# furkanyesiler/acoss

Hardware: AMD Instinct MI355X
Metric: track-pairs/sec on N x N Serra09 Qmax (HPCP, T=2000) (higher is better)
Workload: dtype f32

## Files before the change

acoss_amd/csrc/acx.hip:

```cpp
#include <hip/hip_runtime.h>

#include <chrono>
#include <dlfcn.h>
#include <rccl/rccl.h>

#include <algorithm>
#include <cmath>
#include <cstdio>
#include <cstdlib>
#include <cstring>
#include <string>
#include <vector>

#include "../../include/acx.h"
#include "serra09_kernels.hpp"
#include "serra09_long_kernels.hpp"
#include "serra09_locate_kernels.hpp"
#include "prep_kernels.hpp"
#include "snf_kernels.hpp"
#include "simple_kernels.hpp"
#include "ef_kernels.hpp"
#include "ef_rowstat2_kernels.hpp"
#include "ef_gemm_dma_kernels.hpp"
#include "ef_prep_kernels.hpp"
#include "ftm2d_kernels.hpp"
#include "rank_kernels.hpp"
#include "query_kernels.hpp"
#include "grid.hpp"
#include "serra09_plan.hpp"
#include "device_buffer.hpp"

using acx::PairDesc;
using acx::DeviceBuffer;
using acx::PinnedBuffer;

namespace {

std::string g_create_error;

struct KStat {
    const char *name;
    double ms;
    int64_t launches;
    int64_t cells;
};
enum { KS_OTI = 0, KS_NORMS, KS_BAND, KS_CSM, KS_SEL, KS_QMAX, KS_SIMPLE, KS_EFGEMM, KS_EFSTAT, KS_EFFUSE, KS_EFSW, KS_RANK, KS_TOPK, KS_FTMTILE, KS_QROWS, KS_QTOPK, KS_QRANK, KS_QTOPKL, KS_FTMPAIRS, KS_LOCATE, KS_COUNT };

struct PendingEvent {
    hipEvent_t a, b;
    int stat;
    int64_t cells;
};

struct Serra09Slot {
    std::vector<PairDesc> pd, sorted;
    std::vector<int> perm;
    DeviceBuffer<PairDesc> d_pd;
    DeviceBuffer<float> d_out;
    PinnedBuffer<float> h_out;
    PinnedBuffer<int64_t> h_idx;
    DeviceBuffer<int64_t> d_idx;
    hipEvent_t done = nullptr;
    hipEvent_t cls_ev[8] = {nullptr, nullptr, nullptr, nullptr, nullptr, nullptr, nullptr, nullptr};
    bool busy = false;
    bool on_q = false;
    int B = 0, w = 1;
    int64_t k0 = 0;
    DeviceBuffer<acx_alignment> d_al;
    PinnedBuffer<acx_alignment> h_al;
    std::vector<int64_t> seam_off;
    DeviceBuffer<int64_t> d_seam_off;
    bool al = false;
};

}

struct acx_ctx {
    int device = 0;
    hipStream_t stream = nullptr;
    hipStream_t qstream = nullptr;
    hipStream_t qstream2 = nullptr;
    hipEvent_t q2_done = nullptr;
    std::string err;
    float *d_frames0 = nullptr;
    int64_t *d_toff0 = nullptr;
    std::vector<int64_t> h_off0;
    int pool_tau = 0;
    float *d_frames = nullptr;
    float *d_frot = nullptr;
    _Float16 *d_fh = nullptr;
    float *d_normtab = nullptr;
    int64_t *d_noff = nullptr;
    int normtab_m = 0, normtab_span = -1;
    std::vector<int64_t> h_noff;
    int64_t *d_toff = nullptr;
    float *d_gch = nullptr;
    std::vector<int64_t> h_off;
    int32_t n_tracks = 0, dim = 0;
    DeviceBuffer<double> d_frames64;
    DeviceBuffer<int64_t> d_toff64;
    DeviceBuffer<double> d_prof64;
    DeviceBuffer<double> d_wn64;
    int wn64_L = 0;
    std::vector<int64_t> h_off64;
    int32_t n_tracks64 = 0;
    DeviceBuffer<int32_t> d_pairs;
    DeviceBuffer<double> d_out64;
    float *d_ef[3] = {nullptr, nullptr, nullptr};
    unsigned short *d_efs[3] = {nullptr, nullptr, nullptr};
    int ef_kp[3] = {0, 0, 0};
    float *d_efn[2] = {nullptr, nullptr};
    double *d_efmed = nullptr;
    int64_t *d_efoff = nullptr;
    std::vector<int64_t> h_efoff;
    int32_t ef_ntracks = 0;
    int32_t ef_gemm = ACX_EF_GEMM_DEFAULT;
// ... 551 lines not shown
            if ((int64_t)d.Mq * d.Mr + acx::LOC_STRIP >= ((int64_t)1 << 32))
                return fail(c, ACX_ERR_UNSUPPORTED, "serra09_align: pair " + std::to_string(k) + " has 2^32 cells or more");
        }
    }
    for (int s = 0; s < 2; ++s) {
        if (!c->slot[s].done) ACX_HIP(c, hipEventCreateWithFlags(&c->slot[s].done, hipEventDisableTiming));
        if (c->slot[s].busy) { ACX_HIP(c, hipEventSynchronize(c->slot[s].done)); c->slot[s].busy = false; }
    }

    int64_t k0 = 0;
    for (int batch = 0; k0 < K; ++batch) {
        Serra09Slot &S = c->slot[batch & 1];
        if ((rc = collect_slot(c, S, out, al)) != ACX_OK) return rc;
        std::vector<PairDesc> &pd = S.pd;
        acx::Serra09Arena used;
        const int64_t k = acx::serra09_pack_batch(len, pairs, k0, K, p, dbg != nullptr, limit_floats, pd, used);
        if (k == k0) return fail(c, ACX_ERR_STATE, "serra09: the batch plan made no progress at pair " + std::to_string(k0));
        const int B = (int)pd.size();
        const acx::Serra09Sort srt = acx::serra09_sort_batch(pd, S.sorted, S.perm, p.m);
        const int *key_begin = srt.key_begin, *cls_begin = srt.cls_begin;
        const std::vector<int> &perm = S.perm;
        if (cls_begin[NC] > 0 && (rc = ensure_normtab(c, p)) != ACX_OK) return rc;
        if (cls_begin[NC] > 0 && p.arith == ACX_ARITH_F16X2 && (rc = ensure_f16pool(c)) != ACX_OK) return rc;
        if ((rc = ensure(c, c->d_scratch, (size_t)std::max<int64_t>(used.scratch, 1))) != ACX_OK) return rc;
        if ((rc = ensure(c, c->d_bits, (size_t)std::max<int64_t>(used.bits, 1))) != ACX_OK) return rc;
        if ((rc = ensure(c, c->d_thr, (size_t)used.thr + 64 * 32 + 16)) != ACX_OK) return rc;
        if ((rc = ensure(c, S.d_pd, (size_t)B)) != ACX_OK) return rc;
        if ((rc = ensure(c, S.d_out, (size_t)2 * B)) != ACX_OK) return rc;
        if ((rc = ensure(c, S.h_out, (size_t)2 * B)) != ACX_OK) return rc;
        ACX_HIP(c, hipMemcpyAsync(S.d_pd, pd.data(), sizeof(PairDesc) * B, hipMemcpyHostToDevice, c->stream));
        if (al) {
            int64_t seams = 0;
            S.seam_off.resize((size_t)B);
            for (int k2 = 0; k2 < B; ++k2) { S.seam_off[(size_t)k2] = seams; seams += acx::loc_seam_records(pd[k2].Mq, pd[k2].Mr, p.dp_start); }
            if ((rc = ensure(c, S.d_al, (size_t)B)) != ACX_OK) return rc;
            if ((rc = ensure(c, S.h_al, (size_t)B)) != ACX_OK) return rc;
            if ((rc = ensure(c, S.d_seam_off, (size_t)B)) != ACX_OK) return rc;
            if ((rc = ensure(c, c->d_seam, (size_t)std::max<int64_t>(seams, 1))) != ACX_OK) return rc;
            ACX_HIP(c, hipMemcpyAsync(S.d_seam_off, S.seam_off.data(), sizeof(int64_t) * B, hipMemcpyHostToDevice, c->stream));
        }
        if (dd) {
            if ((rc = ensure(c, S.h_idx, (size_t)B)) != ACX_OK) return rc;
            if ((rc = ensure(c, S.d_idx, (size_t)B)) != ACX_OK) return rc;
            for (int k2 = 0; k2 < B; ++k2) S.h_idx[k2] = dd->idx[k0 + perm[k2]];
            ACX_HIP(c, hipMemcpyAsync(S.d_idx, S.h_idx, sizeof(int64_t) * B, hipMemcpyHostToDevice, c->stream));
        }
        const bool use_q = acx::serra09_switches().qstream && !dbg && !al && !c->prof && cls_begin[NC + 1] == cls_begin[NC];
        if (use_q && !c->qstream) ACX_HIP(c, hipStreamCreateWithFlags(&c->qstream, hipStreamNonBlocking));
        if (use_q && both && !c->qstream2) {
            ACX_HIP(c, hipStreamCreateWithFlags(&c->qstream2, hipStreamNonBlocking));
            ACX_HIP(c, hipEventCreateWithFlags(&c->q2_done, hipEventDisableTiming));
        }
        hipStream_t qs = use_q ? c->qstream : c->stream;
        if (use_q)
            for (int cl = 0; cl < NC; ++cl)
                if (!S.cls_ev[cl]) ACX_HIP(c, hipEventCreateWithFlags(&S.cls_ev[cl], hipEventDisableTiming));
        Serra09Slot &Sprev = c->slot[(batch & 1) ^ 1];
        bool bits_free = !(Sprev.busy && Sprev.on_q);

        {
            ProfScope ps(c, KS_OTI, acx::serra09_extent(pd, 0, B).cells);
            hipLaunchKernelGGL(acx::oti_kernel, dim3((B + 255) / 256), dim3(256), 0, c->stream,
                               S.d_pd, B, c->d_gch, p.oti, p.oti_target, c->d_toff, c->d_noff);
        }
        int64_t cls_cells[NC + 1];
        for (int cl = 0; cl <= NC; ++cl) {
            cls_cells[cl] = 0;
            const int b0 = cls_begin[cl], Bc = cls_begin[cl + 1] - b0;
            if (Bc <= 0) continue;
            const acx::Serra09Extent ce = acx::serra09_extent(pd, b0, b0 + Bc);
            cls_cells[cl] = ce.cells;
            if (cl < NC) {
                bool ok = true;
                for (int cq = 0; cq < NC; ++cq) {
                    const int q0 = key_begin[NC * cl + cq], Bq = key_begin[NC * cl + cq + 1] - q0;
                    if (Bq <= 0) continue;
                    const acx::Serra09Extent qe = acx::serra09_extent(pd, q0, q0 + Bq);
                    ProfScope ps(c, KS_BAND, qe.cells);
                    ok = ok && launch_band(c, p.m, S.d_pd + q0, Bq, qe.Mr, cq, p, 1, 0, dbg ? 1 : 0);
                }
                if (!bits_free) { ACX_HIP(c, hipStreamWaitEvent(c->stream, Sprev.done, 0)); bits_free = true; }
                {
                    ProfScope ps(c, KS_BAND, ce.cells);
                    ok = ok && launch_band(c, p.m, S.d_pd + b0, Bc, ce.Mq, cl, p, 0, dbg ? 1 : 0, dbg ? 1 : 0);
                }
                if (use_q) ACX_HIP(c, hipEventRecord(S.cls_ev[cl], c->stream));
                if (!ok) return fail(c, ACX_ERR_UNSUPPORTED, "serra09: this build of libacx has no band kernel for the requested m");
            } else {
                if (!bits_free) { ACX_HIP(c, hipStreamWaitEvent(c->stream, Sprev.done, 0)); bits_free = true; }
                launch_streaming_class(c, S.d_pd + b0, &pd[b0], Bc, ce, p);
            }
        }
        {
            hipError_t wait_err = hipSuccess;
            auto sweep = [&](bool dmax, float *dst, hipStream_t qs) {
                for (int cl = 0; cl <= NC; ++cl) {
                    const int b0 = cls_begin[cl], Bc = cls_begin[cl + 1] - b0;
                    if (Bc <= 0) continue;
                    if (use_q) { const hipError_t e_ = hipStreamWaitEvent(qs, S.cls_ev[cl], 0); if (e_ != hipSuccess) wait_err = e_; }
                    ProfScope ps(c, KS_QMAX, cls_cells[cl], qs);
                    const acx::Serra09Sweep sw = acx::serra09_sweep(cl);
                    launch_qmax_sweep(qs, S.d_pd + b0, Bc, c->d_bits, c->d_scratch, dst + (size_t)b0 * w, w, p.gamma_o, p.gamma_e, p.dp_start, dmax,
                                      sw.cols, sw.pack);
                }
            };
            if (al) {
                ProfScope ps(c, KS_LOCATE, acx::serra09_extent(pd, 0, B).cells, qs);
                launch_qmax_locate(qs, S.d_pd, B, c->d_bits, c->d_seam, S.d_seam_off, S.d_al, p.gamma_o, p.gamma_e, p.dp_start);
            } else if (both && use_q) {
                sweep(false, S.d_out, qs);
                sweep(true, S.d_out + 1, c->qstream2);
                ACX_HIP(c, hipEventRecord(c->q2_done, c->qstream2));
                ACX_HIP(c, hipStreamWaitEvent(qs, c->q2_done, 0));
            } else if (both) { sweep(false, S.d_out, qs); sweep(true, S.d_out + 1, qs); }
            else sweep(p.dmax != 0, S.d_out, qs);
            ACX_HIP(c, wait_err);
        }
        ACX_LAUNCHES_OK(c);
        if (al) {
            ACX_HIP(c, hipMemcpyAsync(S.h_al, S.d_al, sizeof(acx_alignment) * B, hipMemcpyDeviceToHost, qs));
        } else if (dd) {
            hipLaunchKernelGGL(scatter_scores_kernel, dim3((B + 255) / 256), dim3(256), 0, qs,
                               S.d_out, S.d_idx, dd->base, B, w);
            ACX_HIP(c, hipGetLastError());
        } else {
            ACX_HIP(c, hipMemcpyAsync(S.h_out, S.d_out, sizeof(float) * B * w, hipMemcpyDeviceToHost, qs));
        }
        ACX_HIP(c, hipEventRecord(S.done, qs));
        S.busy = true; S.on_q = use_q; S.B = B; S.w = w; S.k0 = k0; S.al = al != nullptr;

        if (dbg && B >= 1) {
            if ((rc = collect_slot(c, S, out)) != ACX_OK) return rc;
            PairDesc d;
            ACX_HIP(c, hipMemcpy(&d, S.d_pd, sizeof(PairDesc), hipMemcpyDeviceToHost));
            if (dbg->oti) *dbg->oti = d.oti;
            if (dbg->dims) { dbg->dims[0] = d.Mq; dbg->dims[1] = d.Mr; }
            if (dbg->d2)
                ACX_HIP(c, hipMemcpy2D(dbg->d2, sizeof(float) * d.Mr, c->d_scratch + d.offD, sizeof(float) * d.pitchD,
                                       sizeof(float) * d.Mr, d.Mq, hipMemcpyDeviceToHost));
            const float *X = c->d_thr + d.offX;
            if (dbg->thrq) ACX_HIP(c, hipMemcpy(dbg->thrq, X, sizeof(float) * d.Mq, hipMemcpyDeviceToHost));
            if (dbg->thrr) ACX_HIP(c, hipMemcpy(dbg->thrr, X + d.pitchT, sizeof(float) * d.Mr, hipMemcpyDeviceToHost));
            if (dbg->epsq) ACX_HIP(c, hipMemcpy(dbg->epsq, X + d.pitchT + d.pitchD, sizeof(float) * d.Mq, hipMemcpyDeviceToHost));
            if (dbg->epsr) ACX_HIP(c, hipMemcpy(dbg->epsr, X + 2 * d.pitchT + d.pitchD, sizeof(float) * d.Mr, hipMemcpyDeviceToHost));
        }
        k0 = k;
    }
    for (int s = 0; s < 2; ++s)
        if ((rc = collect_slot(c, c->slot[s], out, al)) != ACX_OK) return rc;
    return ACX_OK;
}

}


struct EfDebug { float *csm, *fused; int32_t *oti; int64_t which = 0; };
// ... 580 lines not shown
int acx_abi_version(void) { return ACX_ABI_VERSION; }

int acx_hip_versions(int *build, int *runtime)
{
    if (build) *build = HIP_VERSION;
    int v = 0;
    if (runtime) *runtime = hipRuntimeGetVersion(&v) == hipSuccess ? v : 0;
    return 0;
}

acx_ctx *acx_create(int device, int *err)
{
    auto bad = [&](int code, const std::string &msg) -> acx_ctx * {
        g_create_error = msg;
        if (err) *err = code;
        return nullptr;
    };
    int n = 0;
    hipError_t e = hipGetDeviceCount(&n);
    if (e != hipSuccess || n <= 0) return bad(ACX_ERR_HIP, std::string("no HIP device: ") + hipGetErrorString(e));
    if (device < 0 || device >= n) return bad(ACX_ERR_INVALID, "device index out of range");
    if ((e = hipSetDevice(device)) != hipSuccess) return bad(ACX_ERR_HIP, std::string("hipSetDevice: ") + hipGetErrorString(e));
    hipDeviceProp_t prop;
    if ((e = hipGetDeviceProperties(&prop, device)) != hipSuccess) return bad(ACX_ERR_HIP, std::string("hipGetDeviceProperties: ") + hipGetErrorString(e));
    if (std::string(prop.gcnArchName).rfind("gfx950", 0) != 0)
        return bad(ACX_ERR_HIP, std::string("libacx is built for gfx950 only; device is ") + prop.gcnArchName);
    acx_ctx *c = new acx_ctx();
    c->device = device;
    c->total_mem = prop.totalGlobalMem;
    c->n_cu = prop.multiProcessorCount;
    if ((e = hipStreamCreateWithFlags(&c->stream, hipStreamNonBlocking)) != hipSuccess) {
        delete c;
        return bad(ACX_ERR_HIP, std::string("hipStreamCreate: ") + hipGetErrorString(e));
    }
    if (err) *err = ACX_OK;
    return c;
}

static void comm_release(acx_ctx *c);
static void ftm2d_free_pool(acx_ctx *c);

void acx_destroy(acx_ctx *c)
{
    if (!c) return;
    (void)hipSetDevice(c->device);
    (void)hipStreamSynchronize(c->stream);
    if (c->qstream) (void)hipStreamSynchronize(c->qstream);
    if (c->qstream2) (void)hipStreamSynchronize(c->qstream2);
    comm_release(c);
    drain_profile(c);
    for (hipEvent_t ev : c->event_pool) (void)hipEventDestroy(ev);
    for (Serra09Slot &sl : c->slot) {
        if (sl.done) (void)hipEventDestroy(sl.done);
        for (hipEvent_t ev : sl.cls_ev)
            if (ev) (void)hipEventDestroy(ev);
    }
    for (hipEvent_t ev : c->rank_ev)
        if (ev) (void)hipEventDestroy(ev);
    if (c->q2_done) (void)hipEventDestroy(c->q2_done);
    if (c->qstream) (void)hipStreamDestroy(c->qstream);
    if (c->qstream2) (void)hipStreamDestroy(c->qstream2);
    (void)hipStreamDestroy(c->stream);
    free_pool(c);
    ef_free_pool(c);
    ftm2d_free_pool(c);
    delete c;
}

#ifdef ACX_EF_TIMING
extern "C" int acx_ef_clk(unsigned long long *out, int reset)
{
    if (out && hipMemcpyFromSymbol(out, HIP_SYMBOL(acx::g_ef_clk), sizeof(unsigned long long) * 16) != hipSuccess) return -1;
    if (reset) {
        unsigned long long z[16] = {0};
        if (hipMemcpyToSymbol(HIP_SYMBOL(acx::g_ef_clk), z, sizeof(z)) != hipSuccess) return -1;
    }
    return 0;
}
#endif

const char *acx_last_error(const acx_ctx *c) { return c ? c->err.c_str() : g_create_error.c_str(); }

int acx_set_scratch_limit(acx_ctx *c, int64_t bytes)
{
    if (!c) return ACX_ERR_INVALID;
    c->scratch_limit = bytes < 0 ? 0 : bytes;
    return ACX_OK;
}

int acx_set_nonfinite_policy(acx_ctx *c, int32_t policy)
{
    if (!c) return ACX_ERR_INVALID;
    if (policy != ACX_NONFINITE_REJECT && policy != ACX_NONFINITE_ZERO) return fail(c, ACX_ERR_INVALID, "set_nonfinite_policy: unknown policy");
    c->nonfinite_policy = policy;
    return ACX_OK;
}

int64_t acx_nonfinite_zeroed(const acx_ctx *c) { return c ? c->nf_zeroed : 0; }

static int upload_pool_impl(acx_ctx *c, const float *frames, const int64_t *offsets, int32_t n_tracks, int32_t dim);
static int fill_pool(acx_ctx *c, const float *frames, const int64_t *offsets, int32_t n_tracks, int32_t dim);
static int upload_pool_f64_impl(acx_ctx *c, const double *frames, const int64_t *offsets, int32_t n_tracks, int32_t dim);

int acx_upload_pool(acx_ctx *c, const float *frames, const int64_t *offsets, int32_t n_tracks, int32_t dim)
{
    if (!c) return ACX_ERR_INVALID;
    c->nf_zeroed = 0;
    return upload_pool_impl(c, frames, offsets, n_tracks, dim);
// ... 3083 lines not shown
```

acoss_amd/csrc/serra09_kernels.hpp:

```cpp
#pragma once
#include <hip/hip_runtime.h>
#include <stdint.h>
#include <type_traits>

namespace acx {

constexpr int NBIN = 12;
constexpr int SEL_BINS = 2048;
constexpr int MAX_M = 16;
constexpr int NGUARD = 80;

struct PctPos { float kf, fl, ce; int32_t ilo, ihi, k; };
__host__ __device__ inline PctPos pct_position(int n, float kappa, int pct_mode)
{
    PctPos p;
    p.kf = (n > 1) ? (float)(n - 1) * kappa : (float)n * kappa;
    p.fl = floorf(p.kf); p.ce = ceilf(p.kf);
    int ilo = (int)p.fl, ihi = (int)p.ce;
    ilo = ilo < 0 ? 0 : (ilo > n - 1 ? n - 1 : ilo);
    ihi = ihi < 0 ? 0 : (ihi > n - 1 ? n - 1 : ihi);
    int k = ilo;
    if (pct_mode == 3) {
        k = (int)floorf(p.kf + 0.5f);
        k = k > n - 1 ? n - 1 : k;
// ... 90 lines not shown
    }
    pd[p].oti = best;
}

typedef float f32x4 __attribute__((ext_vector_type(4)));

__device__ __forceinline__ void wave_lds_fence()
{
    __builtin_amdgcn_fence(__ATOMIC_ACQ_REL, "wavefront");
    __builtin_amdgcn_wave_barrier();
}

template <typename Op>
__device__ __forceinline__ int wave_scan_bits(int v, int idn, Op op)
{
    v = op(v, __builtin_amdgcn_update_dpp(idn, v, 0x111, 0xf, 0xf, false));
    v = op(v, __builtin_amdgcn_update_dpp(idn, v, 0x112, 0xf, 0xf, false));
    v = op(v, __builtin_amdgcn_update_dpp(idn, v, 0x114, 0xf, 0xf, false));
    v = op(v, __builtin_amdgcn_update_dpp(idn, v, 0x118, 0xf, 0xf, false));
    v = op(v, __builtin_amdgcn_update_dpp(idn, v, 0x142, 0xa, 0xf, false));
    v = op(v, __builtin_amdgcn_update_dpp(idn, v, 0x143, 0xc, 0xf, false));
    return v;
}
struct OpMinF { __device__ int operator()(int a, int b) const { return __float_as_int(fminf(__int_as_float(a), __int_as_float(b))); } };
struct OpMaxF { __device__ int operator()(int a, int b) const { return __float_as_int(fmaxf(__int_as_float(a), __int_as_float(b))); } };
struct OpAddI { __device__ int operator()(int a, int b) const { return a + b; } };

__device__ __forceinline__ float wave_min(float v)
{
    const int r = wave_scan_bits(__float_as_int(v), __float_as_int(__builtin_inff()), OpMinF());
    return __int_as_float(__builtin_amdgcn_readlane(r, 63));
}
__device__ __forceinline__ float wave_max(float v)
{
    const int r = wave_scan_bits(__float_as_int(v), __float_as_int(-__builtin_inff()), OpMaxF());
    return __int_as_float(__builtin_amdgcn_readlane(r, 63));
}
__device__ __forceinline__ int wave_sum_i(int v)
{
    return __builtin_amdgcn_readlane(wave_scan_bits(v, 0, OpAddI()), 63);
}
__device__ __forceinline__ int wave_incl_scan_i(int v) { return wave_scan_bits(v, 0, OpAddI()); }

template <int SB> struct SelGeom {
    static constexpr int BPL = SB / 64;
    static constexpr int SLOTS = SB + 64 + 16;
    static_assert(SB % 128 == 0, "bins per lane must be even");
    __device__ static __forceinline__ int slot(int b) { return b + b / BPL; }
};
constexpr int SEL_SLOTS = SelGeom<SEL_BINS>::SLOTS;

struct SelectResult { float value; int cnt_le; float next; };

template <int NV, int SB = SEL_BINS>
__device__ __forceinline__ SelectResult wave_select_regs(const float (&x)[NV], int k, unsigned *hist, float *cand,
                                                         unsigned *counter, int lane, bool want_next)
{
    using SG = SelGeom<SB>;
    constexpr int BPL = SG::BPL;
    const float INF = __builtin_inff();
    float mn = INF, mx = -INF;
#pragma unroll
    for (int t = 0; t < NV; ++t) {
        mn = fminf(mn, x[t]);
        mx = fmaxf(mx, (x[t] == INF) ? -INF : x[t]);
    }
    mn = wave_min(mn);
    mx = wave_max(mx);
    int below = 0;
    float result = mn;
    for (int iter = 0; iter < 64; ++iter) {
        if (!(mn < mx)) { result = mn; break; }
        const float scale = (float)SB / (mx - mn);
        for (int b = lane * 4; b < SG::SLOTS; b += 256)
            *reinterpret_cast<uint4 *>(hist + b) = make_uint4(0, 0, 0, 0);
        if (lane == 0) *counter = 0u;
        wave_lds_fence();
        int bins[NV];
#pragma unroll
        for (int t = 0; t < NV; ++t) {
            int b = (int)((x[t] - mn) * scale);
            b = b > SB - 1 ? SB - 1 : b;
            const bool in = x[t] >= mn && x[t] <= mx;
            bins[t] = in ? b : SB;
        }
#pragma unroll
        for (int t = 0; t < NV; ++t)
            __hip_atomic_fetch_add(&hist[SG::slot(bins[t])], 1u, __ATOMIC_RELAXED, __HIP_MEMORY_SCOPE_WORKGROUP);
        wave_lds_fence();
        int hv[BPL];
        int lsum = 0;
#pragma unroll
        for (int e = 0; e < BPL; ++e) { hv[e] = (int)hist[(BPL + 1) * lane + e]; lsum += hv[e]; }
        const int incl = wave_incl_scan_i(lsum);
        const int target = k - below;
        const unsigned long long m = __ballot(incl > target);
        const int L = __ffsll((long long)m) - 1;
        const int excl = incl - lsum;
        int binsel_v = 0, cum_v = 0, cnt_v = 0;
        {
            int run = excl;
#pragma unroll
            for (int e = 0; e < BPL; ++e) {
                const bool here = cnt_v == 0 && run + hv[e] > target;
                binsel_v = here ? BPL * lane + e : binsel_v;
                cum_v = here ? run : cum_v;
                cnt_v = here ? hv[e] : cnt_v;
                run += hv[e];
            }
        }
        const int binsel = __builtin_amdgcn_readlane(binsel_v, L);
        const int cum = __builtin_amdgcn_readlane(cum_v, L);
        const int cnt = __builtin_amdgcn_readlane(cnt_v, L);
        if (cnt <= 64) {
#pragma unroll
            for (int t = 0; t < NV; ++t) {
                const bool hit = bins[t] == binsel;
                if (__ballot(hit) != 0ull) {
                    if (hit) {
                        unsigned pos = __hip_atomic_fetch_add(counter, 1u, __ATOMIC_RELAXED, __HIP_MEMORY_SCOPE_WORKGROUP);
                        cand[pos & 63u] = x[t];
                    }
                }
            }
            wave_lds_fence();
            const float mine = (lane < cnt) ? cand[lane] : INF;
            int rank = 0;
#pragma unroll 1
            for (int t = 0; t < cnt; ++t) {
                const float o = __int_as_float(__builtin_amdgcn_readlane(__float_as_int(mine), t));
                rank += (o < mine || (o == mine && t < lane)) ? 1 : 0;
            }
            const int want = target - cum;
            const unsigned long long hitm = __ballot(lane < cnt && rank == want);
            const int src = __ffsll((long long)hitm) - 1;
            result = __int_as_float(__builtin_amdgcn_readlane(__float_as_int(mine), src));
            wave_lds_fence();
            break;
        }
        float nmn = INF, nmx = -INF;
#pragma unroll
        for (int t = 0; t < NV; ++t) {
            if (bins[t] == binsel) { nmn = fminf(nmn, x[t]); nmx = fmaxf(nmx, x[t]); }
        }
        below += cum;
        mn = wave_min(nmn);
        mx = wave_max(nmx);
        result = mn;
        wave_lds_fence();
    }
    SelectResult res{result, 0, INF};
    if (want_next) {
        int cle = 0;
        float nx = INF;
#pragma unroll
        for (int t = 0; t < NV; ++t) {
            cle += (x[t] <= result) ? 1 : 0;
            nx = fminf(nx, (x[t] > result) ? x[t] : INF);
        }
        res.cnt_le = wave_sum_i(cle);
        res.next = wave_min(nx);
    }
// ... 635 lines not shown

#ifdef ACX_TIMING
#define ACX_STAMP_PARM , StampT &tstamp_
#define ACX_STAMP_ARG , tstamp_
#else
#define ACX_STAMP_PARM
#define ACX_STAMP_ARG
#endif
template <int NV, int ROLE>
__device__ __forceinline__ void band_row_tail(float (&xr)[NV], float *smem, int wave, int lane, int row, int MA, int MB,
                                              int cshift, const PairDesc &P, float *__restrict__ thr,
                                              unsigned long long *__restrict__ bits, const PctPos &pp, int pct_mode,
                                              int inclusive, int want_eps ACX_STAMP_PARM)
{
    using RG = RowGeom<NV>;
    constexpr int ROWP = RG::ROWP, FBINS = RG::FBINS, FCOPIES = RG::FCOPIES, PBINS = RG::PBINS, PGRP = RG::PGRP, GBINS = RG::GBINS;
    constexpr bool HIST_IN_ROW = RG::HIST_IN_ROW;
    constexpr float PDELTA = RG::PDELTA;
    constexpr int CH = NV / 4;
    constexpr int role = ROLE;
    const float INF = __builtin_inff();
    const int hist_off = RG::hist_off(wave);
    if (row >= MA) return;
    const int n = MB;
    const float kf = pp.kf, fl = pp.fl, ce = pp.ce;
    const int ilo = pp.ilo, ihi = pp.ihi, k = pp.k;
    const bool interp = (pct_mode == 0 || pct_mode == 1);
    float *myrow = smem + wave * ROWP;
    float slo, shi;
    typedef __attribute__((address_space(3))) void lds_void;
    const unsigned hist_addr = (unsigned)(uintptr_t)(lds_void *)(smem + hist_off);
    const bool use_pivot = (ihi + 2) * 9 <= n;
    auto zero_hist = [&](int bins) {
        float *h = smem + hist_off;
        for (int q = 0; q < bins / 256; ++q) *reinterpret_cast<float4 *>(h + 256 * q + 4 * lane) = make_float4(0.f, 0.f, 0.f, 0.f);
        wave_lds_fence();
    };
    if constexpr (HIST_IN_ROW) zero_hist(use_pivot ? PBINS : FBINS);
    bool done = false;
    const int end_valid = MB + cshift;
    const bool lane_has_data = lane * NV < end_valid;
    if (use_pivot) {
        const int g0 = (lane & ~(PGRP - 1)) * NV;
        const bool group_full = g0 >= cshift && g0 + PGRP * NV <= end_valid;
        done = wave_select_pivot<NV, PBINS, PGRP>(xr, k, interp && ihi != ilo, hist_addr, myrow, lane, slo, shi,
                                                  lane_has_data, group_full, PDELTA);
        if (!done) zero_hist(FBINS);
    }
    if (!done)
        done = wave_select_fast<NV, FBINS, FCOPIES>(xr, k, interp && ihi != ilo, hist_addr, myrow, lane, slo, shi, lane_has_data);
    if (!done) {
        unsigned *ghist = reinterpret_cast<unsigned *>(myrow) + 64;
        unsigned *counter = reinterpret_cast<unsigned *>(myrow) + 64 + SelGeom<GBINS>::SLOTS;
        const SelectResult sr = wave_select_regs<NV, GBINS>(xr, k, ghist, myrow, counter, lane, interp);
        slo = sr.value;
        shi = (interp && ihi != ilo && sr.cnt_le <= ihi) ? sr.next : sr.value;
    }
    ACX_STAMP(5);
    ACX_ABL_EXIT(3, slo + shi);
    typedef float f32x4_u __attribute__((ext_vector_type(4), aligned(4)));
    constexpr bool TC_VIA_LDS = NV >= 32;
    f32x4_u tcg[CH];
    if constexpr (TC_VIA_LDS) {
        if (role == 0 && bits) {
            asm volatile("" ::: "memory");
            const float *tc = thr + P.offX + P.pitchT - cshift + 4 * lane;
#pragma unroll
            for (int q = 0; q < CH; ++q) tcg[q] = *reinterpret_cast<const f32x4_u *>(tc + 256 * q);
        }
    }
    const bool weights_ok = interp && ihi == ilo + 1 && inclusive && fl >= 1.0f && (ce - kf) >= 0.00390625f && (kf - fl) >= 0.00390625f;
    if (!want_eps && weights_ok && shi < INF && (shi - slo) > shi * 0.000244140625f) {
        ACX_STAMP(6);
        ACX_ABL_EXIT(4, slo);
        if (lane == 0) (thr + P.offX)[role ? P.pitchT + row : row] = slo;
        band_row_bits<NV, ROLE, TC_VIA_LDS>(xr, tcg, slo, myrow, lane, row, MB, cshift, P, thr, bits);
        ACX_STAMP(7);
        return;
    }
    float dlo, dhi;
    const float eps = percentile_eps2(slo, shi, pct_mode, ilo, ihi, kf, fl, ce, dlo, dhi);
    float thr_row;
    if (inclusive && dlo <= eps && eps < dhi) thr_row = slo;
    else thr_row = d2_threshold(eps, inclusive);
    ACX_STAMP(6);
    float *X = thr + P.offX;
    if (lane == 0) {
        const int o = role ? P.pitchT + row : row;
        X[o] = thr_row;
        X[P.pitchT + P.pitchD + o] = eps;
    }
    band_row_bits<NV, ROLE, TC_VIA_LDS>(xr, tcg, thr_row, myrow, lane, row, MB, cshift, P, thr, bits);
    ACX_STAMP(7);
}

constexpr int band_waves_per_simd(int m, int v4, int arith = 0) { return (v4 <= 2 && m <= 9) ? ACX_NARROW_WAVES : ((v4 <= 4 && m <= 9) ? (arith ? 6 : ACX_MID_WAVES) : 4); }
template <int M, int V4, int ROLE, bool WD2 = false, int ARITH = 0>
__global__ __launch_bounds__(BAND_THREADS, band_waves_per_simd(M, V4, ARITH)) void band_kernel(const float *__restrict__ frot,
                                                            const int64_t *__restrict__ toff,
                                                            const float *__restrict__ normtab,
                                                            const int64_t *__restrict__ noff,
                                                            const PairDesc *__restrict__ pd,
                                                            float *__restrict__ scratch,
                                                            float *__restrict__ thr,
                                                            unsigned long long *__restrict__ bits,
                                                            float kappa, int pct_mode, int inclusive, int oti_target, int want_eps)
{
    constexpr bool write_d2 = WD2;
    using G = BandGeom<M, V4, ARITH>;
    constexpr int role = ROLE;
    constexpr int NV = 4 * V4;
    constexpr int NSTEP = NV / 8;
    using RG = RowGeom<NV>;
    constexpr int LNP = RG::LNP, ROWP = RG::ROWP, FBINS = RG::FBINS;
    constexpr bool HIST_IN_ROW = RG::HIST_IN_ROW;
    constexpr int SWEEP_FLOATS = 8 * G::AROWS * G::SP;
    constexpr int LDS_FLOATS = SWEEP_FLOATS > RG::TAIL_FLOATS ? SWEEP_FLOATS : RG::TAIL_FLOATS;
    __shared__ __attribute__((aligned(4096))) float smem[LDS_FLOATS];

    const int bid_x = blockIdx.x, bid_y = blockIdx.y;
    const PairDesc P = pd[bid_y];
    const int MA = role ? P.Mr : P.Mq, MB = role ? P.Mq : P.Mr;
    const int TA = role ? P.Tr : P.Tq, TB = role ? P.Tq : P.Tr;
    const int i0 = bid_x * BAND;
    if (i0 >= MA) return;
    const int tid = threadIdx.x, lane = tid & 63;
    const int wave = __builtin_amdgcn_readfirstlane(tid >> 6);
    const bool rows_are_ref = role == 1;
    const int rota = (rows_are_ref == (oti_target == 0)) ? P.oti : 0;
    const int rotb = (rows_are_ref == (oti_target == 0)) ? 0 : P.oti;
    const float *nrow = normtab + (role ? P.nr : P.nq) + (int64_t)rota * (MA + NGUARD);
    const float *ncol = normtab + (role ? P.nq : P.nr) + (int64_t)rotb * (MB + NGUARD);
    const float INF = __builtin_inff();
    const float PADV = INF;

    const int lr = lane & 15, lk = lane >> 4;
    int c0a = lk - rota; if (c0a < 0) c0a += NBIN;
    int c0b = lk - rotb; if (c0b < 0) c0b += NBIN;
    constexpr unsigned PB = ARITH ? (unsigned)FH * 2u : (unsigned)FROT * 4u;
    const unsigned offA = ARITH ? (unsigned)(((c0a >> 2) * 4 + (c0a & 3)) * 16) : (unsigned)(((c0a >> 2) * NBIN + (c0a & 3) * 3) * 4);
    const unsigned offB = ARITH ? (unsigned)(((c0b >> 2) * 4 + (c0b & 3)) * 16) : (unsigned)(((c0b >> 2) * NBIN + (c0b & 3) * 3) * 4);
    const char *pool_b = reinterpret_cast<const char *>(frot);
    const char *fra = pool_b + (role ? P.fr : P.fq) * (int64_t)PB + offA;
    const __amdgpu_buffer_rsrc_t rsB =
        __builtin_amdgcn_make_buffer_rsrc((void *)(pool_b + ((role ? P.fq : P.fr) - 8) * (int64_t)PB), 0, -1, 0x00020000);
    const unsigned voffB = offB + (unsigned)lr * PB;
    const char *frb = pool_b + (role ? P.fq : P.fr) * (int64_t)PB + offB;
    typedef float f32x3 __attribute__((ext_vector_type(3)));
    typedef f32x3 f32x3_u __attribute__((aligned(4)));
    typedef unsigned u32x3 __attribute__((ext_vector_type(3)));
    typedef u32x3 u32x3_u __attribute__((aligned(4)));
    typedef unsigned u32x4v __attribute__((ext_vector_type(4)));
    typedef _Float16 f16x8 __attribute__((ext_vector_type(8)));
    typedef _Float16 f16x4 __attribute__((ext_vector_type(4)));
    float areg[G::NRT][3];
    f16x8 ah8[G::NRT], ah9[G::NRT];
#pragma unroll
    for (int ta = 0; ta < G::NRT; ++ta) {
        int f = i0 + 16 * ta + lr;
// ... 196 lines not shown
            const int a = idx / npad, j = MB + idx - a * npad;
            if (i0 + a < MA) D[a * pitchD + j] = INF;
        }
    }
    ACX_STAMP(0);
#ifdef ACX_ABL
    { float keep_ = 0.0f;
      for (int a = 0; a < BAND; ++a) for (int st = 0; st < NSTEP; ++st) keep_ += xv[a][st];
      ACX_ABL_EXIT(1, keep_); }
#endif
    __syncthreads();
    ACX_STAMP(1);
    constexpr int CH = NV / 4;
    constexpr int LPT = 64 / NV == 0 ? 1 : 64 / NV;
    static_assert(NV == 8 || NV == 16 || NV == 32, "row owners hold 8, 16 or 32 consecutive positions");
    {
        const int wl = lane + 4 * (lane / NV);
#pragma unroll
        for (int st = 0; st < NSTEP; ++st) {
            float *dst = smem + tile_of(st) * (LPT * LNP) + wl;
#pragma unroll
            for (int a = 0; a < BAND; ++a) dst[a * ROWP] = xv[a][st];
        }
    }
    if constexpr (!HIST_IN_ROW) {
        float *h = smem + RG::hist_off(wave);
#pragma unroll
        for (int q = 0; q < FBINS / 256; ++q) *reinterpret_cast<float4 *>(h + 256 * q + 4 * lane) = make_float4(0.f, 0.f, 0.f, 0.f);
    }
    ACX_STAMP(2);
    __syncthreads();
    ACX_STAMP(3);
    float xr[NV];
    {
        const float *mine = smem + wave * ROWP + lane * LNP;
#pragma unroll
        for (int j = 0; j < CH; ++j) {
            const float4 v = *reinterpret_cast<const float4 *>(mine + 4 * j);
            xr[4 * j + 0] = v.x; xr[4 * j + 1] = v.y; xr[4 * j + 2] = v.z; xr[4 * j + 3] = v.w;
        }
    }

    asm volatile("s_waitcnt lgkmcnt(0)" ::: "memory");
    ACX_STAMP(4);
#ifdef ACX_ABL
    { float keep_ = 0.0f;
      for (int t = 0; t < NV; ++t) keep_ += xr[t];
      ACX_ABL_EXIT(2, keep_); }
#endif
    band_row_tail<NV, ROLE>(xr, smem, wave, lane, i0 + wave, MA, MB, (BAND - 1) - wave, P, thr, role == 0 ? bits : nullptr,
                            pp, pct_mode, inclusive, want_eps ACX_STAMP_ARG);
}

template <bool EQG, bool DMAX, int CPL>
__device__ __forceinline__ void qmax_cells(unsigned wraw, unsigned colmask, unsigned wprev, unsigned wleft,
                                           float l1a, float l1b, float l2a, float p1a, float p1b, float p2a,
                                           const float (&QA)[CPL], float (&QB)[CPL],
                                           const float (&PA)[EQG ? 1 : CPL], float (&PB)[EQG ? 1 : CPL],
                                           float go, float ge, float &best)
{
    const unsigned w = wraw & colmask;
#pragma unroll
    for (int e = CPL - 1; e >= 0; --e) {
        const bool r = (w >> e) & 1u;
        float x3 = 0.0f, x4 = 0.0f;
        if constexpr (DMAX) {
            x3 = ((wprev >> e) & 1u) ? 1.0f : 0.0f;
            x4 = ((wleft >> e) & 1u) ? 1.0f : 0.0f;
        }
        const float c2 = (e >= 1) ? QA[e - 1] : l1a;
        float c3 = (e >= 1) ? QB[e - 1] : l2a;
        float c4 = (e >= 2) ? QA[e - 2] : (e == 1 ? l1a : l1b);
        if constexpr (DMAX) { c3 += x3; c4 += x4; }
        const float mx = fmaxf(fmaxf(c2, c3), c4);
        float q;
        if constexpr (EQG) {
            const int m = __builtin_amdgcn_sbfe((int)w, e, 1);
            const float t = __int_as_float((m & __float_as_int(1.0f)) | (~m & __float_as_int(-go)));
            q = fmaxf(mx + t, 0.0f);
        } else {
            const float a2 = (e >= 1) ? PA[e - 1] : p1a;
            float a3 = (e >= 1) ? PB[e - 1] : p2a;
            float a4 = (e >= 2) ? PA[e - 2] : (e == 1 ? p1a : p1b);
            if constexpr (DMAX) { a3 += x3; a4 += x4; }
            const float vgap = fmaxf(fmaxf(fmaxf(a2, a3), a4), 0.0f);
            q = r ? (mx + 1.0f) : vgap;
        }
        if constexpr (DMAX) { if (!((colmask >> e) & 1u)) q = 0.0f; }
        QB[e] = q;
        if constexpr (!EQG) PB[e] = q - ((DMAX ? (((wraw >> e) & 1u) != 0u) : r) ? go : ge);
    }
#pragma unroll
    for (int e = 0; e < CPL; e += 2) best = fmaxf(best, fmaxf(QB[e], QB[e + 1]));
}

template <bool EQG, bool DMAX, int CPL>
__global__ __launch_bounds__(64) void qmax_bits_kernel(const PairDesc *__restrict__ pd,
                                                       const unsigned long long *__restrict__ bits,
                                                       float *__restrict__ out, int out_stride,
                                                       float go, float ge, int dp_start)
{
    const int lane = threadIdx.x;
    const PairDesc P = pd[blockIdx.x];
    int Me = P.Mq, Ne = P.Mr;
    if (dp_start == 3) { Me -= 1; Ne -= 1; }
    const int ndw = 2 * P.nw;
// ... 301 lines not shown
```

acoss_amd/csrc/serra09_plan.hpp:

```cpp
#pragma once
#include <algorithm>
#include <cstdint>
#include <cstdlib>
#include <vector>

#include "../../include/acx.h"
#include "serra09_kernels.hpp"

namespace acx {

inline int serra09_tiles(int M) { return (M + BAND - 1 + 63) / 64; }

inline int64_t serra09_round_up(int64_t v, int64_t m) { return (v + m - 1) / m * m; }

inline int serra09_embed_len(int T, int m, int tau, int embed_full)
{
    const int span = embed_full ? (m - 1) * tau : m * tau;
    const int L = T - span;
    if (L <= 0) return 0;
    return (L + tau - 1) / tau;
}

constexpr int SERRA09_NC = 5;
struct Serra09Class {
    int tiles;
    int band_m9, band_m10, band_f16;
    int cols, pack;
};
constexpr Serra09Class SERRA09_CLASS[SERRA09_NC] = {
    {4, ACX_SERRA09_FAMILY_BAND2_4ROWS, ACX_SERRA09_FAMILY_BAND_2, ACX_SERRA09_FAMILY_BAND_2, 8, 4},
    {8, ACX_SERRA09_FAMILY_BAND2_2ROWS, ACX_SERRA09_FAMILY_BAND_2, ACX_SERRA09_FAMILY_BAND_2, 8, 2},
    {12, ACX_SERRA09_FAMILY_BAND2_MID, ACX_SERRA09_FAMILY_BAND_4, ACX_SERRA09_FAMILY_BAND_4, 16, 1},
    {16, ACX_SERRA09_FAMILY_BAND_4, ACX_SERRA09_FAMILY_BAND_4, ACX_SERRA09_FAMILY_BAND_4, 16, 1},
    {32, ACX_SERRA09_FAMILY_BAND_8, ACX_SERRA09_FAMILY_BAND_8, ACX_SERRA09_FAMILY_BAND_8, 32, 1},
};

inline int serra09_row_class(int M)
{
    const int nd = serra09_tiles(M);
    int cl = 0;
    while (cl < SERRA09_NC && nd > SERRA09_CLASS[cl].tiles) ++cl;
    return cl;
}

struct Serra09Switches {
    int band2;
    bool multi, qstream;
};
inline const Serra09Switches &serra09_switches()
{
    static const Serra09Switches s = [] {
        auto off = [](const char *name) { const char *e = getenv(name); return e && e[0] == '0'; };
        const char *b = getenv("ACX_BAND2");
        return Serra09Switches{(b && b[0] >= '0' && b[0] <= '2') ? b[0] - '0' : 3, !off("ACX_QMAX_MULTI"), !off("ACX_QMAX_STREAM")};
    }();
    return s;
}

inline int serra09_band_family(int cl, int m, int arith)
{
    const Serra09Class &c = SERRA09_CLASS[cl];
    if (arith == ACX_ARITH_F16X2) return c.band_f16;
    if (m > 9) return c.band_m10;
    const int keep = serra09_switches().band2;
    switch (c.band_m9) {
    case ACX_SERRA09_FAMILY_BAND2_4ROWS: return keep >= 3 ? c.band_m9 : (keep >= 1 ? ACX_SERRA09_FAMILY_BAND2_2ROWS : ACX_SERRA09_FAMILY_BAND_2);
    case ACX_SERRA09_FAMILY_BAND2_2ROWS: return keep >= 1 ? c.band_m9 : ACX_SERRA09_FAMILY_BAND_2;
    case ACX_SERRA09_FAMILY_BAND2_MID: return keep >= 2 ? c.band_m9 : ACX_SERRA09_FAMILY_BAND_4;
    default: return c.band_m9;
    }
}

struct Serra09Sweep { int cols, pack; };
inline Serra09Sweep serra09_sweep(int cl)
{
    if (cl >= SERRA09_NC) return Serra09Sweep{0, 1};
    return Serra09Sweep{SERRA09_CLASS[cl].cols, serra09_switches().multi ? SERRA09_CLASS[cl].pack : 1};
}

inline const char *serra09_family_name(int family, int m)
{
    const bool lo = m <= 9;
    switch (family) {
    case ACX_SERRA09_FAMILY_BAND2_4ROWS: return "band2_kernel<M, B2_NV, 16>";
    case ACX_SERRA09_FAMILY_BAND2_2ROWS: return "band2_kernel<M, B2_NV, 32>";
    case ACX_SERRA09_FAMILY_BAND2_MID: return "band2_kernel<M, B2_NV_MID, 32>";
    case ACX_SERRA09_FAMILY_BAND_2: return lo ? "band_kernel<M<=9, 2>" : "band_kernel<M>=10, 2>";
    case ACX_SERRA09_FAMILY_BAND_4: return lo ? "band_kernel<M<=9, 4>" : "band_kernel<M>=10, 4>";
    case ACX_SERRA09_FAMILY_BAND_8: return lo ? "band_kernel<M<=9, 8>" : "band_kernel<M>=10, 8>";
    case ACX_SERRA09_FAMILY_STREAMING: return "csm_long_kernel + rowsel_long_kernel";
    default: return nullptr;
    }
}

struct Serra09Lengths {
    const int64_t *off;
    int32_t n_tracks;
    int tau;
    int operator()(int t) const
    {
        const int64_t T = off[t + 1] - off[t];
        return (int)(tau == 1 ? T : (T + tau - 1) / tau);
    }
};

struct Serra09Need {
    int64_t D, L;
    int64_t bits;
    int64_t thr;
    int64_t floats() const { return D + L + 2 * bits; }
// ... 111 lines not shown
```

Baseline: 105,600.

## Split row classes into chunks so qmax sweeps overlap band kernels

```diff
diff --git a/acoss_amd/csrc/acx.hip b/acoss_amd/csrc/acx.hip
--- a/acoss_amd/csrc/acx.hip
+++ b/acoss_amd/csrc/acx.hip
@@ -61,7 +61,7 @@
     PinnedBuffer<int64_t> h_idx;
     DeviceBuffer<int64_t> d_idx;
     hipEvent_t done = nullptr;
-    hipEvent_t cls_ev[8] = {nullptr, nullptr, nullptr, nullptr, nullptr, nullptr, nullptr, nullptr};
+    std::vector<hipEvent_t> chunk_ev;
     bool busy = false;
     bool on_q = false;
     int B = 0, w = 1;
@@ -719,9 +719,8 @@
             ACX_HIP(c, hipEventCreateWithFlags(&c->q2_done, hipEventDisableTiming));
         }
         hipStream_t qs = use_q ? c->qstream : c->stream;
-        if (use_q)
-            for (int cl = 0; cl < NC; ++cl)
-                if (!S.cls_ev[cl]) ACX_HIP(c, hipEventCreateWithFlags(&S.cls_ev[cl], hipEventDisableTiming));
+        struct Chunk { int cl, b0, n; int64_t cells; };
+        std::vector<Chunk> chunks;
         Serra09Slot &Sprev = c->slot[(batch & 1) ^ 1];
         bool bits_free = !(Sprev.busy && Sprev.on_q);
 
@@ -730,45 +729,55 @@
             hipLaunchKernelGGL(acx::oti_kernel, dim3((B + 255) / 256), dim3(256), 0, c->stream,
                                S.d_pd, B, c->d_gch, p.oti, p.oti_target, c->d_toff, c->d_noff);
         }
-        int64_t cls_cells[NC + 1];
         for (int cl = 0; cl <= NC; ++cl) {
-            cls_cells[cl] = 0;
             const int b0 = cls_begin[cl], Bc = cls_begin[cl + 1] - b0;
             if (Bc <= 0) continue;
-            const acx::Serra09Extent ce = acx::serra09_extent(pd, b0, b0 + Bc);
-            cls_cells[cl] = ce.cells;
             if (cl < NC) {
-                bool ok = true;
-                for (int cq = 0; cq < NC; ++cq) {
-                    const int q0 = key_begin[NC * cl + cq], Bq = key_begin[NC * cl + cq + 1] - q0;
-                    if (Bq <= 0) continue;
-                    const acx::Serra09Extent qe = acx::serra09_extent(pd, q0, q0 + Bq);
-                    ProfScope ps(c, KS_BAND, qe.cells);
-                    ok = ok && launch_band(c, p.m, S.d_pd + q0, Bq, qe.Mr, cq, p, 1, 0, dbg ? 1 : 0);
+                const int nch = use_q ? acx::serra09_chunks(Bc) : 1;
+                for (int ch = 0; ch < nch; ++ch) {
+                    const int c0 = acx::serra09_chunk_begin(b0, Bc, nch, ch), c1 = acx::serra09_chunk_begin(b0, Bc, nch, ch + 1);
+                    const acx::Serra09Extent ce = acx::serra09_extent(pd, c0, c1);
+                    bool ok = true;
+                    for (int cq = 0; cq < NC; ++cq) {
+                        const int q0 = std::max(c0, key_begin[NC * cl + cq]), Bq = std::min(c1, key_begin[NC * cl + cq + 1]) - q0;
+                        if (Bq <= 0) continue;
+                        const acx::Serra09Extent qe = acx::serra09_extent(pd, q0, q0 + Bq);
+                        ProfScope ps(c, KS_BAND, qe.cells);
+                        ok = ok && launch_band(c, p.m, S.d_pd + q0, Bq, qe.Mr, cq, p, 1, 0, dbg ? 1 : 0);
+                    }
+                    if (!bits_free) { ACX_HIP(c, hipStreamWaitEvent(c->stream, Sprev.done, 0)); bits_free = true; }
+                    {
+                        ProfScope ps(c, KS_BAND, ce.cells);
+                        ok = ok && launch_band(c, p.m, S.d_pd + c0, c1 - c0, ce.Mq, cl, p, 0, dbg ? 1 : 0, dbg ? 1 : 0);
+                    }
+                    if (use_q) {
+                        if (S.chunk_ev.size() <= chunks.size()) {
+                            hipEvent_t ev = nullptr;
+                            ACX_HIP(c, hipEventCreateWithFlags(&ev, hipEventDisableTiming));
+                            S.chunk_ev.push_back(ev);
+                        }
+                        ACX_HIP(c, hipEventRecord(S.chunk_ev[chunks.size()], c->stream));
+                    }
+                    chunks.push_back(Chunk{cl, c0, c1 - c0, ce.cells});
+                    if (!ok) return fail(c, ACX_ERR_UNSUPPORTED, "serra09: this build of libacx has no band kernel for the requested m");
                 }
-                if (!bits_free) { ACX_HIP(c, hipStreamWaitEvent(c->stream, Sprev.done, 0)); bits_free = true; }
-                {
-                    ProfScope ps(c, KS_BAND, ce.cells);
-                    ok = ok && launch_band(c, p.m, S.d_pd + b0, Bc, ce.Mq, cl, p, 0, dbg ? 1 : 0, dbg ? 1 : 0);
-                }
-                if (use_q) ACX_HIP(c, hipEventRecord(S.cls_ev[cl], c->stream));
-                if (!ok) return fail(c, ACX_ERR_UNSUPPORTED, "serra09: this build of libacx has no band kernel for the requested m");
             } else {
+                const acx::Serra09Extent ce = acx::serra09_extent(pd, b0, b0 + Bc);
                 if (!bits_free) { ACX_HIP(c, hipStreamWaitEvent(c->stream, Sprev.done, 0)); bits_free = true; }
                 launch_streaming_class(c, S.d_pd + b0, &pd[b0], Bc, ce, p);
+                chunks.push_back(Chunk{cl, b0, Bc, ce.cells});
             }
         }
         {
             hipError_t wait_err = hipSuccess;
             auto sweep = [&](bool dmax, float *dst, hipStream_t qs) {
-                for (int cl = 0; cl <= NC; ++cl) {
-                    const int b0 = cls_begin[cl], Bc = cls_begin[cl + 1] - b0;
-                    if (Bc <= 0) continue;
-                    if (use_q) { const hipError_t e_ = hipStreamWaitEvent(qs, S.cls_ev[cl], 0); if (e_ != hipSuccess) wait_err = e_; }
-                    ProfScope ps(c, KS_QMAX, cls_cells[cl], qs);
-                    const acx::Serra09Sweep sw = acx::serra09_sweep(cl);
-                    launch_qmax_sweep(qs, S.d_pd + b0, Bc, c->d_bits, c->d_scratch, dst + (size_t)b0 * w, w, p.gamma_o, p.gamma_e, p.dp_start, dmax,
-                                      sw.cols, sw.pack);
+                for (size_t ci = 0; ci < chunks.size(); ++ci) {
+                    const Chunk &ck = chunks[ci];
+                    if (use_q) { const hipError_t e_ = hipStreamWaitEvent(qs, S.chunk_ev[ci], 0); if (e_ != hipSuccess) wait_err = e_; }
+                    ProfScope ps(c, KS_QMAX, ck.cells, qs);
+                    const acx::Serra09Sweep sw = acx::serra09_sweep(ck.cl);
+                    launch_qmax_sweep(qs, S.d_pd + ck.b0, ck.n, c->d_bits, c->d_scratch, dst + (size_t)ck.b0 * w, w, p.gamma_o, p.gamma_e, p.dp_start,
+                                      dmax, sw.cols, sw.pack);
                 }
             };
             if (al) {
@@ -1455,8 +1464,7 @@
     for (hipEvent_t ev : c->event_pool) (void)hipEventDestroy(ev);
     for (Serra09Slot &sl : c->slot) {
         if (sl.done) (void)hipEventDestroy(sl.done);
-        for (hipEvent_t ev : sl.cls_ev)
-            if (ev) (void)hipEventDestroy(ev);
+        for (hipEvent_t ev : sl.chunk_ev) (void)hipEventDestroy(ev);
     }
     for (hipEvent_t ev : c->rank_ev)
         if (ev) (void)hipEventDestroy(ev);
diff --git a/acoss_amd/csrc/serra09_kernels.hpp b/acoss_amd/csrc/serra09_kernels.hpp
--- a/acoss_amd/csrc/serra09_kernels.hpp
+++ b/acoss_amd/csrc/serra09_kernels.hpp
@@ -166,7 +166,7 @@
 
 struct SelectResult { float value; int cnt_le; float next; };
 
-template <int NV, int SB = SEL_BINS>
+template <int NV, int SB = SEL_BINS, bool LEAN = false>
 __device__ __forceinline__ SelectResult wave_select_regs(const float (&x)[NV], int k, unsigned *hist, float *cand,
                                                          unsigned *counter, int lane, bool want_next)
 {
@@ -217,11 +217,12 @@
 #pragma unroll
             for (int e = 0; e < BPL; ++e) {
                 const bool here = cnt_v == 0 && run + hv[e] > target;
-                binsel_v = here ? BPL * lane + e : binsel_v;
+                binsel_v = here ? (LEAN ? e : BPL * lane + e) : binsel_v;
                 cum_v = here ? run : cum_v;
                 cnt_v = here ? hv[e] : cnt_v;
                 run += hv[e];
             }
+            if constexpr (LEAN) binsel_v += BPL * lane;
         }
         const int binsel = __builtin_amdgcn_readlane(binsel_v, L);
         const int cum = __builtin_amdgcn_readlane(cum_v, L);
@@ -963,7 +964,7 @@
     if (!done) {
         unsigned *ghist = reinterpret_cast<unsigned *>(myrow) + 64;
         unsigned *counter = reinterpret_cast<unsigned *>(myrow) + 64 + SelGeom<GBINS>::SLOTS;
-        const SelectResult sr = wave_select_regs<NV, GBINS>(xr, k, ghist, myrow, counter, lane, interp);
+        const SelectResult sr = wave_select_regs<NV, GBINS, NV >= 32 && ROLE == 1>(xr, k, ghist, myrow, counter, lane, interp);
         slo = sr.value;
         shi = (interp && ihi != ilo && sr.cnt_le <= ihi) ? sr.next : sr.value;
     }
@@ -1006,16 +1007,14 @@
 }
 
 constexpr int band_waves_per_simd(int m, int v4, int arith = 0) { return (v4 <= 2 && m <= 9) ? ACX_NARROW_WAVES : ((v4 <= 4 && m <= 9) ? (arith ? 6 : ACX_MID_WAVES) : 4); }
-template <int M, int V4, int ROLE, bool WD2 = false, int ARITH = 0>
-__global__ __launch_bounds__(BAND_THREADS, band_waves_per_simd(M, V4, ARITH)) void band_kernel(const float *__restrict__ frot,
-                                                            const int64_t *__restrict__ toff,
-                                                            const float *__restrict__ normtab,
-                                                            const int64_t *__restrict__ noff,
-                                                            const PairDesc *__restrict__ pd,
-                                                            float *__restrict__ scratch,
-                                                            float *__restrict__ thr,
-                                                            unsigned long long *__restrict__ bits,
-                                                            float kappa, int pct_mode, int inclusive, int oti_target, int want_eps)
+template <int M, int V4, int ROLE, bool WD2, int ARITH>
+__device__ __forceinline__ void band_kernel_body(const float *__restrict__ frot,
+                                                 const float *__restrict__ normtab,
+                                                 const PairDesc *__restrict__ pd,
+                                                 float *__restrict__ scratch,
+                                                 float *__restrict__ thr,
+                                                 unsigned long long *__restrict__ bits,
+                                                 int pct_mode, int inclusive, int oti_target, int want_eps)
 {
     constexpr bool write_d2 = WD2;
     using G = BandGeom<M, V4, ARITH>;
@@ -1318,6 +1317,26 @@
                             pp, pct_mode, inclusive, want_eps ACX_STAMP_ARG);
 }
 
+constexpr int BAND_COL_VGPRS = 112;
+constexpr bool band_leaves_sweep_room(int m, int v4, int role, bool wd2, int arith) { return m <= 9 && v4 >= 8 && role == 1 && !wd2 && arith == 0; }
+#define ACX_BAND_KERNEL_PARMS const float *__restrict__ frot, const int64_t *__restrict__ toff, const float *__restrict__ normtab, \
+                              const int64_t *__restrict__ noff, const PairDesc *__restrict__ pd, float *__restrict__ scratch, \
+                              float *__restrict__ thr, unsigned long long *__restrict__ bits, float kappa, int pct_mode, int inclusive, \
+                              int oti_target, int want_eps
+template <int M, int V4, int ROLE, bool WD2 = false, int ARITH = 0, std::enable_if_t<!band_leaves_sweep_room(M, V4, ROLE, WD2, ARITH), int> = 0>
+__global__ __launch_bounds__(BAND_THREADS, band_waves_per_simd(M, V4, ARITH)) void band_kernel(ACX_BAND_KERNEL_PARMS)
+{
+    band_kernel_body<M, V4, ROLE, WD2, ARITH>(frot, normtab, pd, scratch, thr, bits, pct_mode, inclusive, oti_target, want_eps);
+}
+template <int M, int V4, int ROLE, bool WD2 = false, int ARITH = 0, std::enable_if_t<band_leaves_sweep_room(M, V4, ROLE, WD2, ARITH), int> = 1>
+__global__ __launch_bounds__(BAND_THREADS, band_waves_per_simd(M, V4, ARITH)) __attribute__((amdgpu_num_vgpr(56)))
+void band_kernel(ACX_BAND_KERNEL_PARMS)
+{
+    static_assert(BAND_COL_VGPRS == 2 * 56, "the attribute's literal");
+    band_kernel_body<M, V4, ROLE, WD2, ARITH>(frot, normtab, pd, scratch, thr, bits, pct_mode, inclusive, oti_target, want_eps);
+}
+#undef ACX_BAND_KERNEL_PARMS
+
 template <bool EQG, bool DMAX, int CPL>
 __device__ __forceinline__ void qmax_cells(unsigned wraw, unsigned colmask, unsigned wprev, unsigned wleft,
                                            float l1a, float l1b, float l2a, float p1a, float p1b, float p2a,
diff --git a/acoss_amd/csrc/serra09_plan.hpp b/acoss_amd/csrc/serra09_plan.hpp
--- a/acoss_amd/csrc/serra09_plan.hpp
+++ b/acoss_amd/csrc/serra09_plan.hpp
@@ -43,19 +43,39 @@
     return cl;
 }
 
+constexpr int SERRA09_SUBBATCH_MIN = 1024;
+constexpr int SERRA09_MAX_CHUNKS = 8;
 struct Serra09Switches {
     int band2;
     bool multi, qstream;
+    int chunks;
+    int chunk_min;
 };
 inline const Serra09Switches &serra09_switches()
 {
     static const Serra09Switches s = [] {
         auto off = [](const char *name) { const char *e = getenv(name); return e && e[0] == '0'; };
+        auto num = [](const char *name, long lo, long hi, long dflt) {
+            const char *e = getenv(name);
+            if (!e || !(e[0] >= '0' && e[0] <= '9')) return (int)dflt;
+            const long v = strtol(e, nullptr, 10);
+            return (int)(v < lo ? lo : (v > hi ? hi : v));
+        };
         const char *b = getenv("ACX_BAND2");
-        return Serra09Switches{(b && b[0] >= '0' && b[0] <= '2') ? b[0] - '0' : 3, !off("ACX_QMAX_MULTI"), !off("ACX_QMAX_STREAM")};
+        return Serra09Switches{(b && b[0] >= '0' && b[0] <= '2') ? b[0] - '0' : 3, !off("ACX_QMAX_MULTI"), !off("ACX_QMAX_STREAM"),
+                               num("ACX_SERRA09_CHUNKS", 0, SERRA09_MAX_CHUNKS, -1), num("ACX_SERRA09_CHUNK_MIN", 1, 65535, SERRA09_SUBBATCH_MIN)};
     }();
     return s;
 }
+
+inline int serra09_chunks(int pairs)
+{
+    const Serra09Switches &s = serra09_switches();
+    if (s.chunks == 0 || pairs < 2 * (int64_t)s.chunk_min) return 1;
+    const int c = s.chunks > 0 ? s.chunks : std::min(4, std::max(2, pairs / s.chunk_min));
+    return std::min(c, pairs);
+}
+inline int serra09_chunk_begin(int b0, int pairs, int c, int ch) { return b0 + (int)((int64_t)pairs * ch / c); }
 
 inline int serra09_band_family(int cl, int m, int arith)
 {
```

After: 103,300. 0.979x the previous value.
